# avianphysics/avian

Measured on NVIDIA H100. Metric: physics steps/sec on 100k-cube stack (broad phase + solver stage per step), higher is better.
Workload: dtype f32

## Files before the change

### avian_b200/csrc/solver_dev.cuh

```cuda
#pragma once
#include <cuda_pipeline.h>

#include "../../include/avian_b200.h"
#include "avn_math.cuh"

namespace avn {

enum { CP_N = 0, CP_T1 = 1, CP_TV = 2, CP_IDX = 3, CP_PT0 = 4, CP_PLANES = CP_PT0 + 3 * AVN_MAX_MANIFOLD_POINTS };
#define CP_ROW(k, r) (CP_PT0 + 3 * (k) + (r))
enum { CI_NP_MASK = 0x7, CI_ZERO1 = 1 << 4, CI_ZERO2 = 1 << 5, CI_NONDYN = 1 << 6, CI_TANGENT = 1 << 7,
       CI_VER1 = 1 << 8, CI_VER2 = 1 << 9 };
enum { BF_LOCK_MASK = 0x3f, BF_HAS_SOLVER_BODY = 1 << 8, BF_KINEMATIC = 1 << 9, BF_GYRO = 1 << 10, BF_DYNAMIC = 1 << 11,
       BF_CUSTOM_VEL = 1 << 12, BF_CUSTOM_POS = 1 << 13, BF_DOMINANCE_SHIFT = 16 };

enum { JP_IDX = 0,
       JP_R1 = 1,
       JP_R2 = 2,
       JP_CD = 3,
       JP_RD = 4,
       JP_A1 = 5,
       JP_A2 = 6,
       JP_B1 = 7,
       JP_B2 = 8,
       JP_LP = 9,
// ... 2 lines not shown
       JP_PLANES = 12 };

template <class S>
struct Soft { S bias, mass_scale, impulse_scale; };

template <class S>
struct DevSolver {
    int B, M, P, Mpad, J, Jpad, n_levels;
    int m_color_off[AVN_GRAPH_COLOR_COUNT + 1];
    int color_off[AVN_GRAPH_COLOR_COUNT + 1];
    int color_len[AVN_GRAPH_COLOR_COUNT];
    int wave;
    unsigned int* ver;
    int* deg;
    int* stamp;
    int substeps, iters, rest_iters, fast_trig, match_contacts;
    S h, dt, max_overlap_speed, warm_coeff, rest_threshold, joint_force_rhs;
    S gx, gy, gz;
    Soft<S> soft_dyn, soft_nondyn;
    const uint8_t* kind; const uint8_t* locked; const int8_t* dominance; const uint8_t* integ_flags;
    const S* position; const S* rotation; const S* linvel; const S* angvel; const S* inv_mass; const S* inv_inertia_local;
    const S* com; const S* lin_damp; const S* ang_damp; const S* grav_scale; const S* lin_acc; const S* ang_acc;
    const S* max_lin; const S* max_ang;
    S* out_position; S* out_rotation; S* out_linvel; S* out_angvel;
    Vec4<S>* vel; Vec4<S>* dlt; Vec4<S>* inr; Vec4<S>* itg; Vec4<S>* pre;
    const int* m_body1; const int* m_body2; const S* m_normal; const S* m_friction; const S* m_restitution; const S* m_tanvel;
    const uint32_t* m_point_begin; const uint32_t* m_point_end; const uint32_t* m_src;
    const S* p_anchor1; const S* p_anchor2; const S* p_penetration; const S* p_normal_speed;
    const S* p_ws_normal; const S* p_ws_tangent;
    const S* p_in_normal_impulse;
// ... 191 lines not shown
                                              V3<S> r1, V3<S> r2, V3<S> imp) {
    v1 = v1 - cmul(imp, in1.inv_mass);
    w1 = w1 - smul(in1.ii, cross(r1, imp));
    v2 = v2 + cmul(imp, in2.inv_mass);
    w2 = w2 + smul(in2.ii, cross(r2, imp));
}

enum { FLAG_RESTITUTION = 0, FLAG_WAVE = 1, FLAG_WORDS = 4 };
#ifdef AVN_WAVE_TRACE
#define AVN_TRACE_T(var) const long long var = clock64()
#define AVN_TRACE_ADD(d, i, v) do { if ((threadIdx.x & 31) == 0) atomicAdd(reinterpret_cast<unsigned long long*>((d).any_restitution + FLAG_WORDS) + (i), (unsigned long long)(v)); } while (0)
#else
#define AVN_TRACE_T(var)
#define AVN_TRACE_ADD(d, i, v)
#endif
__device__ __forceinline__ unsigned events_per_substep(int k, int iters) { return 2u + unsigned(2 + iters) * unsigned(k); }
enum { WV_IV = 0, WV_WARM = 1, WV_SOLVE = 2, WV_IP = 3, WV_RELAX = 4 };
__device__ __forceinline__ unsigned wave_event(int kind, int it, int s, int iters, int k, int r) {
    unsigned base = unsigned(s) * events_per_substep(k, iters);
    switch (kind) {
        case WV_IV: return base;
        case WV_WARM: return base + 1u + r;
        case WV_SOLVE: return base + 1u + unsigned(1 + it) * k + r;
        case WV_IP: return base + 1u + unsigned(1 + iters) * k;
        default: return base + 2u + unsigned(1 + iters) * k + r;
    }
}
__device__ __forceinline__ unsigned ld_acquire(const unsigned* p) {
    unsigned v;
    asm volatile("ld.acquire.gpu.global.u32 %0, [%1];" : "=r"(v) : "l"(p) : "memory");
    return v;
}
__device__ __forceinline__ void st_relaxed(unsigned* p, unsigned v) { asm volatile("st.relaxed.gpu.global.u32 [%0], %1;" ::"l"(p), "r"(v) : "memory"); }
__device__ __forceinline__ void fence_acq_rel() { asm volatile("fence.acq_rel.gpu;" ::: "memory"); }
__device__ __forceinline__ Vec4<float> ld4_cg(const Vec4<float>* p) {
    float4 v = __ldcg(reinterpret_cast<const float4*>(p));
    return mk4<float>(v.x, v.y, v.z, v.w);
}
__device__ __forceinline__ Vec4<double> ld4_cg(const Vec4<double>* p) {
    double2 a = __ldcg(reinterpret_cast<const double2*>(p)), b = __ldcg(reinterpret_cast<const double2*>(p) + 1);
// ... 18 lines not shown
    if (need2) st_relaxed(ver + b2, e2 + 1u);
}

constexpr int STAGE_ROWS = 3 * AVN_MAX_MANIFOLD_POINTS;
template <class S> __device__ __forceinline__ Vec4<S>* stage_base() {
    extern __shared__ __align__(32) unsigned char avn_stage_raw[];
    return reinterpret_cast<Vec4<S>*>(avn_stage_raw);
}
__device__ __forceinline__ void stage_copy(Vec4<float>* dst, const Vec4<float>* src) { __pipeline_memcpy_async(dst, src, 16); }
__device__ __forceinline__ void stage_copy(Vec4<double>* dst, const Vec4<double>* src) {
    __pipeline_memcpy_async(dst, src, 16);
    __pipeline_memcpy_async(reinterpret_cast<char*>(dst) + 16, reinterpret_cast<const char*>(src) + 16, 16);
}
template <class S> __host__ __device__ constexpr size_t stage_bytes(int threads, int max_points = AVN_MAX_MANIFOLD_POINTS) {
    return size_t(4 * max_points) * threads * sizeof(Vec4<S>);
}

template <class S, int PASS, int MAXP = AVN_MAX_MANIFOLD_POINTS>
__device__ __forceinline__ void contact_item(const DevSolver<S>& d, int slot) {
    const size_t MP = size_t(d.Mpad);
    Vec4<S>* c = d.cst + slot;
    Vec4<S> hidx = ld4(&c[CP_IDX * MP]);
    const int info = as_int(hidx.z);
    const int np = info & CI_NP_MASK;
    if (np == 0) return;
    const int b1 = as_int(hidx.x), b2 = as_int(hidx.y);
    Vec4<S> hn = mk4<S>(0, 0, 0, 0), ht1 = hn, htv = hn;
    BodyInertia<S> in1 = zero_inertia<S>(), in2 = zero_inertia<S>();
    Vec4<S> PC[MAXP];
    constexpr bool SOLVE = (PASS == PASS_SOLVE_BIAS || PASS == PASS_RELAX);
// ... 140 lines not shown
            if (k < np) pc_store(pc_ptr(d, k, slot), PC[k]);
    }
    if (!(info & CI_ZERO1)) {
        st4(&d.vel[2 * b1], mk4<S>(v1.x, v1.y, v1.z, S(0)));
        st4(&d.vel[2 * b1 + 1], mk4<S>(w1.x, w1.y, w1.z, S(0)));
    }
    if (!(info & CI_ZERO2)) {
        st4(&d.vel[2 * b2], mk4<S>(v2.x, v2.y, v2.z, S(0)));
        st4(&d.vel[2 * b2 + 1], mk4<S>(w2.x, w2.y, w2.z, S(0)));
    }
#undef ROW_A
#undef ROW_B
#undef ROW_D
}

template <class S, int PASS, int MAXP>
__device__ __forceinline__ void wave_contact_item(const DevSolver<S>& d, int slot, int s, int it, bool relax) {
    constexpr bool SOLVE = PASS == PASS_SOLVE_BIAS;
    relax = SOLVE && relax;
    const size_t MP = size_t(d.Mpad);
    const Vec4<S>* c = d.cst + slot;
    const Vec4<S> hidx = ld4(&c[CP_IDX * MP]);
    const int info = as_int(hidx.z);
    const int np = info & CI_NP_MASK;
    const int b1 = as_int(hidx.x), b2 = as_int(hidx.y);
    Vec4<S>* const stage = stage_base<S>() + threadIdx.x;
    const int T = blockDim.x;
#define ROW_A(k) stage[(3 * (k) + 0) * T]
#define ROW_B(k) stage[(3 * (k) + 1) * T]
#define ROW_D(k) stage[(3 * (k) + 2) * T]
#define ROW_PC(k) stage[(3 * MAXP + (k)) * T]
    Vec4<S> hn = mk4<S>(0, 0, 0, 0), ht1 = hn, htv = hn;
    BodyInertia<S> in1 = zero_inertia<S>(), in2 = zero_inertia<S>();
    if (np != 0) {
        hn = ld4(&c[CP_N * MP]);
        ht1 = ld4(&c[CP_T1 * MP]);
        if (SOLVE) htv = ld4(&c[CP_TV * MP]);
        if (!(info & CI_ZERO1)) in1 = unpack_inertia(ld4(&d.inr[2 * b1]), ld4(&d.inr[2 * b1 + 1]));
        if (!(info & CI_ZERO2)) in2 = unpack_inertia(ld4(&d.inr[2 * b2]), ld4(&d.inr[2 * b2 + 1]));
#pragma unroll 1
        for (int k = 0; k < np; ++k) {
            stage_copy(&ROW_A(k), &c[size_t(CP_ROW(k, 0)) * MP]);
            stage_copy(&ROW_B(k), &c[size_t(CP_ROW(k, 1)) * MP]);
            if (SOLVE && (info & CI_TANGENT)) stage_copy(&ROW_D(k), &c[size_t(CP_ROW(k, 2)) * MP]);
        }
    }
    __pipeline_commit();
    const bool ver1 = np != 0 && (info & CI_VER1), ver2 = np != 0 && (info & CI_VER2);
    const int rk = as_int(hidx.w);
    const int k1 = (rk >> 8) & 0xff, k2 = (rk >> 24) & 0xff;
    const int kind = SOLVE ? (relax ? WV_RELAX : WV_SOLVE) : WV_WARM;
    const unsigned e1 = wave_event(kind, it, s, d.iters, k1, rk & 0xff);
    const unsigned e2 = wave_event(kind, it, s, d.iters, k2, (rk >> 16) & 0xff);
    int* const watchdog = d.any_restitution + FLAG_WAVE;
    const V3<S> n = xyz(hn), t1 = xyz(ht1);
    const Soft<S> soft = (info & CI_NONDYN) ? d.soft_nondyn : d.soft_dyn;
    unsigned biased_points = 0;
    unsigned seen1 = 0u, seen2 = 0u;

    if (SOLVE) {
        AVN_TRACE_T(t_d0);
        const int sd = relax ? s : s - 1;
        if (sd >= 0)
            wave_wait<false>(d.ver, ver1, b1, wave_event(WV_IP, 0, sd, d.iters, k1, 0) + 1u, ver2, b2, wave_event(WV_IP, 0, sd, d.iters, k2, 0) + 1u,
                             watchdog, &seen1, &seen2);
        __pipeline_wait_prior(0);
        if (np != 0) {
            const Vec4<S> dp1 = ld4_cg(&d.dlt[2 * b1]), dq1 = ld4_cg(&d.dlt[2 * b1 + 1]);
            const Vec4<S> dp2 = ld4_cg(&d.dlt[2 * b2]), dq2 = ld4_cg(&d.dlt[2 * b2 + 1]);
            Q4<S> q1; q1.x = dq1.x; q1.y = dq1.y; q1.z = dq1.z; q1.w = dq1.w;
            Q4<S> q2; q2.x = dq2.x; q2.y = dq2.y; q2.z = dq2.z; q2.w = dq2.w;
            const V3<S> delta_translation = xyz(dp2) - xyz(dp1);
#pragma unroll
            for (int k = 0; k < MAXP; ++k) {
                if (k >= np) break;
// ... 18 lines not shown
    wave_wait(d.ver, ver1 && seen1 != e1, b1, e1, ver2 && seen2 != e2, b2, e2, watchdog);
    AVN_TRACE_ADD(d, 0, clock64() - t_w0);
    if (np == 0) return;
    AVN_TRACE_T(t_l0);
    const Vec4<S> l1 = ld4_cg(&d.vel[2 * b1]), a1 = ld4_cg(&d.vel[2 * b1 + 1]);
    const Vec4<S> l2 = ld4_cg(&d.vel[2 * b2]), a2 = ld4_cg(&d.vel[2 * b2 + 1]);
    {
        Vec4<S> pc[MAXP];
#pragma unroll
        for (int k = 0; k < MAXP; ++k)
            if (k < np) pc[k] = pc_load<true>(pc_ptr(d, k, slot));
#pragma unroll
        for (int k = 0; k < MAXP; ++k)
            if (k < np) ROW_PC(k) = pc[k];
    }
    if (!SOLVE) __pipeline_wait_prior(0);
#ifdef AVN_WAVE_TRACE
    if ((l1.x + a1.x + l2.x + a2.x) == S(1.2345e33)) d.any_restitution[1] = 2;
    AVN_TRACE_T(t_c0);
    AVN_TRACE_ADD(d, 1, t_c0 - t_l0);
#endif
    V3<S> v1 = xyz(l1), w1 = xyz(a1), v2 = xyz(l2), w2 = xyz(a2);
    const V3<S> t2 = cross(t1, n);

    if (!SOLVE) {
#pragma unroll 1
        for (int k = 0; k < np; ++k) {
            const Vec4<S> PAk = ROW_A(k), PBk = ROW_B(k), pck = ROW_PC(k);
            V3<S> r1 = xyz(PAk), r2 = xyz(PBk);
            S tx = (info & CI_TANGENT) ? pck.z : S(0), ty = (info & CI_TANGENT) ? pck.w : S(0);
            V3<S> p = d.warm_coeff * ((pck.x * n + tx * t1) + ty * t2);
            apply_impulse(v1, w1, v2, w2, in1, in2, r1, r2, p);
        }
    } else {
        const bool tangent = (info & CI_TANGENT) != 0;
#pragma unroll 1
        for (int k = 0; k < np; ++k) {
            const Vec4<S> PAk = ROW_A(k), PBk = ROW_B(k);
            Vec4<S> pck = ROW_PC(k);
            V3<S> r1 = xyz(PAk), r2 = xyz(PBk);
            V3<S> relv = (v2 + cross(w2, r2)) - (v1 + cross(w1, r1));
            S vn = dot(relv, n);
            S acc = pck.x;
            const S C = ((biased_points >> k) & 1u) ? soft.impulse_scale * acc : S(0);
            S impulse = -PBk.w * (vn + PAk.w) - C;
            S new_impulse = avn_max(acc + impulse, S(0));
            impulse = new_impulse - acc;
            pck.x = new_impulse;
            pck.y = pck.y + new_impulse;
// ... 47 lines not shown
    if (!(info & CI_ZERO2)) {
        st4(&d.vel[2 * b2], mk4<S>(v2.x, v2.y, v2.z, S(0)));
        st4(&d.vel[2 * b2 + 1], mk4<S>(w2.x, w2.y, w2.z, S(0)));
    }
    wave_publish(d.ver, ver1, b1, e1, ver2, b2, e2);
#ifdef AVN_WAVE_TRACE
    AVN_TRACE_ADD(d, 3, clock64() - t_s0);
    AVN_TRACE_ADD(d, 4, 1);
#endif
#undef ROW_A
#undef ROW_B
#undef ROW_D
#undef ROW_PC
}

template <class S, bool WAVE = false>
__device__ __forceinline__ void integrate_velocity_item(const DevSolver<S>& d, int i, int s = 0) {
    const bool in_range = i < d.B;
    int f = 0;
    if (in_range) f = as_int(ld4(&d.inr[2 * i]).y);
    const bool live = in_range && (f & BF_HAS_SOLVER_BODY);
    const bool integrate = live && !(f & BF_CUSTOM_VEL) && !(f & BF_KINEMATIC), gyro = integrate && (f & BF_GYRO);
    Vec4<S> li = mk4<S>(0, 0, 0, 0), ai = li;
    Q4<S> rot0; rot0.x = rot0.y = rot0.z = rot0.w = S(0);
    Sym3<S> il; il.m00 = il.m01 = il.m02 = il.m11 = il.m12 = il.m22 = S(0);
    if (integrate) { li = ld4(&d.itg[2 * i]); ai = ld4(&d.itg[2 * i + 1]); }
    if (gyro) {
        rot0 = ldq(d.rotation, i);
        il.m00 = d.inv_inertia_local[6 * i]; il.m01 = d.inv_inertia_local[6 * i + 1]; il.m02 = d.inv_inertia_local[6 * i + 2];
        il.m11 = d.inv_inertia_local[6 * i + 3]; il.m12 = d.inv_inertia_local[6 * i + 4]; il.m22 = d.inv_inertia_local[6 * i + 5];
    }
    const S max_lin = live && d.max_lin ? d.max_lin[i] : S(0), max_ang = live && d.max_ang ? d.max_ang[i] : S(0);
    const int bnd = live && d.bnd_of ? d.bnd_of[i] : -1;
    unsigned e = 0;
    if (WAVE) {
        if (live) e = wave_event(WV_IV, 0, s, d.iters, d.deg[i], 0);
        wave_wait(d.ver, live, i, e, false, 0, 0u, d.any_restitution + 1);
    }
    if (!live) return;
    Vec4<S> l = ldm<WAVE>(&d.vel[2 * i]), a = ldm<WAVE>(&d.vel[2 * i + 1]);
    V3<S> v = xyz(l), w = xyz(a);
    bool touched = false;
    if (integrate) {
        v = v * li.w;
        w = w * ai.w;
        v = v + xyz(li);
        w = w + xyz(ai);
        if (gyro) {
            Vec4<S> dq4 = ldm<WAVE>(&d.dlt[2 * i + 1]);
            Q4<S> dq; dq.x = dq4.x; dq.y = dq4.y; dq.z = dq4.z; dq.w = dq4.w;
            Q4<S> rot = qmul(dq, rot0);
            V3<S> lw = qrot(qconj(rot), w);
            Sym3<S> tensor = sym_inverse_or_zero(il);
            V3<S> L = smul(tensor, lw);
// ... 4 lines not shown
            } else {
                Ln = Ln * avn_sqrt(len2(L) / l2);
                w = qrot(rot, smul(il, Ln));
            }
        }
        touched = true;
    }
    if (d.max_lin) {
        S l2 = len2(v);
        if (avn_finite(max_lin) && l2 > max_lin * max_lin) { v = v * (max_lin / avn_sqrt(l2)); touched = true; }
    }
    if (d.max_ang) {
        S l2 = len2(w);
        if (avn_finite(max_ang) && l2 > max_ang * max_ang) { w = w * (max_ang / avn_sqrt(l2)); touched = true; }
    }
    if (touched) {
        st4(&d.vel[2 * i], mk4<S>(v.x, v.y, v.z, S(0)));
        st4(&d.vel[2 * i + 1], mk4<S>(w.x, w.y, w.z, S(0)));
    }
    if (bnd >= 0) {
        st4(&d.vel_ref[2 * bnd], mk4<S>(v.x, v.y, v.z, S(0)));
        st4(&d.vel_ref[2 * bnd + 1], mk4<S>(w.x, w.y, w.z, S(0)));
    }
    if (WAVE) wave_publish(d.ver, true, i, e, false, 0, 0u);
}

template <class S, bool WAVE = false>
__device__ __forceinline__ void integrate_position_item(const DevSolver<S>& d, int i, int s = 0) {
    const bool in_range = i < d.B;
    int f = 0;
    if (in_range) f = as_int(ld4(&d.inr[2 * i]).y);
    const bool live = in_range && (f & BF_HAS_SOLVER_BODY);
    unsigned e = 0;
    if (WAVE) {
        if (live) e = wave_event(WV_IP, 0, s, d.iters, d.deg[i], 0);
        wave_wait(d.ver, live, i, e, false, 0, 0u, d.any_restitution + 1);
    }
    if (!live) return;
    if (f & BF_CUSTOM_POS) {
// ... 26 lines not shown
    if (info & CI_VER1) { bad |= atomicExch(&d.stamp[b1], colour + 1) == colour + 1; r1 = atomicAdd(&d.deg[b1], 1); }
    if (info & CI_VER2) { bad |= atomicExch(&d.stamp[b2], colour + 1) == colour + 1; r2 = atomicAdd(&d.deg[b2], 1); }
    if (bad || r1 > 0xfe || r2 > 0xfe) d.any_restitution[1] = WAVE_BAD_COLOURING;
    hidx.w = int_as(S(0), (r1 & 0xff) | ((r2 & 0xff) << 16));
    st4(&c[CP_IDX * MP], hidx);
}
template <class S>
__device__ __forceinline__ void wave_pack_item(const DevSolver<S>& d, int slot) {
    const size_t MP = size_t(d.Mpad);
    Vec4<S>* c = d.cst + slot;
    Vec4<S> hidx = ld4(&c[CP_IDX * MP]);
    const int info = as_int(hidx.z);
    if ((info & CI_NP_MASK) == 0) return;
    const int b1 = as_int(hidx.x), b2 = as_int(hidx.y);
    int rk = as_int(hidx.w);
    if (info & CI_VER1) rk |= (d.deg[b1] & 0xff) << 8;
    if (info & CI_VER2) rk |= (d.deg[b2] & 0xff) << 24;
    hidx.w = int_as(S(0), rk);
    st4(&c[CP_IDX * MP], hidx);
}

template <class S>
__device__ __forceinline__ void writeback_body_item(const DevSolver<S>& d, int i) {
    Vec4<S> ia = ld4(&d.inr[2 * i]);
    int f = as_int(ia.y);
    V3<S> pos = ldv3(d.position, i);
    Q4<S> rot = ldq(d.rotation, i);
    V3<S> lv = ldv3(d.linvel, i), av = ldv3(d.angvel, i);
    if (f & BF_HAS_SOLVER_BODY) {
        Vec4<S> l = ld4(&d.vel[2 * i]), a = ld4(&d.vel[2 * i + 1]);
        Vec4<S> dp = ld4(&d.dlt[2 * i]), dq4 = ld4(&d.dlt[2 * i + 1]);
        V3<S> com = ldv3_or0(d.com, i);
        V3<S> old_com = qrot(rot, com);
        Q4<S> dq; dq.x = dq4.x; dq.y = dq4.y; dq.z = dq4.z; dq.w = dq4.w;
// ... 39 lines not shown
```

### avian_b200/csrc/solver_host.cu

```cuda
#include <algorithm>
#include <cmath>
#include <cstdlib>
#include <cstring>

#include "context.hpp"
#include "joint_schedule.hpp"
#include "solver_kernels.cuh"

namespace avn {

namespace {

template <class S>
Soft<S> softness(S damping_ratio, S hz, S delta_secs) {
    S double_damping_ratio = S(2) * damping_ratio;
    S angular_frequency = S(6.283185307179586476925286766559) * hz;
    S a1 = double_damping_ratio + angular_frequency * delta_secs;
    S a2 = angular_frequency * delta_secs * a1;
    S a3 = S(1) / (S(1) + a2);
    Soft<S> s;
    s.bias = angular_frequency / a1;
    s.mass_scale = a2 * a3;
    s.impulse_scale = a3;
    return s;
// ... 160 lines not shown
    ErrorSink* err_;
    uint32_t cfg_flags_;
    int sm_count_ = 132;
    bool coop_ok_ = false, use_mega_ = true, use_wave_ = true, l2_persist_ = false;
    size_t l2_persist_bytes_ = 0, l2_window_max_ = 0;
    int mega_grid_ = 0, mega_bps_ = 3, mega_maxp_ = 0, mega_sel_bps_ = 0;
    bool force_wave_ = false;

    template <int MAXP> const void* mega_variant(int bps) const {
        switch (bps) {
            case 2: return (const void*)step_megakernel<S, 2, MAXP>;
            case 4: return (const void*)step_megakernel<S, 4, MAXP>;
            default: return (const void*)step_megakernel<S, 3, MAXP>;
        }
    }
    static size_t mega_smem_bytes(int maxp) { return stage_bytes<S>(MEGA_BLOCK, maxp); }
    bool select_megakernel(int max_points, int bps = 0) {
        const int maxp = max_points <= 1 ? 1 : AVN_MAX_MANIFOLD_POINTS;
        if (bps == 0) bps = mega_bps_;
        if (maxp == mega_maxp_ && bps == mega_sel_bps_) return mega_grid_ > 0;
        mega_maxp_ = maxp;
        mega_sel_bps_ = bps;
        mega_fn_ = maxp == 1 ? mega_variant<1>(bps) : mega_variant<AVN_MAX_MANIFOLD_POINTS>(bps);
        const size_t smem = mega_smem_bytes(maxp);
        int per_sm = 0;
        mega_grid_ = 0;
        if (cudaFuncSetAttribute(mega_fn_, cudaFuncAttributeMaxDynamicSharedMemorySize, int(smem)) == cudaSuccess &&
            cudaOccupancyMaxActiveBlocksPerMultiprocessor(&per_sm, mega_fn_, MEGA_BLOCK, smem) == cudaSuccess && per_sm > 0)
            mega_grid_ = per_sm * sm_count_;
        else
            (void)cudaGetLastError();
// ... 369 lines not shown

        hm_ = *mc;
        if (mc->device_list) {
            host_any_restitution_ = mc->list_restitution;
        } else if (mc->reuse_graph) {
            host_any_restitution_ = graph_restitution_;
        } else {
            host_any_restitution_ = false;
            const S* r = static_cast<const S*>(mc->restitution);
            for (size_t i = 0; i < mc->M; ++i) host_any_restitution_ |= (r[i] != S(0));
            graph_restitution_ = host_any_restitution_;
        }
    }
    {
        auto up256 = [](size_t x) { return (x + 255) & ~size_t(255); };
        const size_t vel_b = up256(state_bytes), dlt_b = up256(state_bytes), ver_b = up256((B + 1) * sizeof(unsigned)), deg_b = up256(2 * (B + 1) * sizeof(int));
        const size_t planes_b = have_m_ ? size_t(CP_PLANES) * d.Mpad * sizeof(Vec4<S>) : 0;
        const size_t pcr_b = have_m_ ? up256(size_t(AVN_MAX_MANIFOLD_POINTS) * d.Mpad * sizeof(Vec4<S>)) : 0;
        AVN_CUDA(hot_.ensure(vel_b + dlt_b + ver_b + deg_b + pcr_b + planes_b + 256));
        char* base = hot_.as<char>();
        d.vel = reinterpret_cast<Vec4<S>*>(base); base += vel_b;
        d.dlt = reinterpret_cast<Vec4<S>*>(base); base += dlt_b;
        d.ver = reinterpret_cast<unsigned*>(base); base += ver_b;
        d.deg = reinterpret_cast<int*>(base); d.stamp = d.deg + (B + 1); base += deg_b;
        d.pcr = have_m_ ? reinterpret_cast<Vec4<S>*>(base) : nullptr; base += pcr_b;
        d.cst = have_m_ ? reinterpret_cast<Vec4<S>*>(base) : nullptr;
        hot_bytes_ = vel_b + dlt_b + ver_b + deg_b + pcr_b;
    }
    have_j_ = false;
    if (js) {
        size_t J = 0;
        for (int t = 0; t < AVN_JOINT_TYPE_COUNT; ++t) J += js->types[t].count;
        if (J > 0) {
            if ((st = build_joint_schedule(*bc, *js)) != AVN_OK) return st;
            have_j_ = true;
            for (int t = 0; t < AVN_JOINT_TYPE_COUNT; ++t) {
                const AvnJointColumns& jc = js->types[t];
                const size_t n = jc.count;
                const void* cols[12] = {jc.local_anchor1, jc.local_anchor2, jc.local_basis1, jc.local_basis2, jc.axis, jc.limit_min,
                                        jc.limit_max, jc.limit2_min, jc.limit2_max, jc.compliance0, jc.compliance1, jc.compliance2};
                const size_t width[12] = {3, 3, 4, 4, 3, 1, 1, 1, 1, 1, 1, 1};
// ... 69 lines not shown
    if (prepare) step_bps_ = mega_bps_;
    mega = mega && select_megakernel(max_np_, step_bps_);
    if (prepare) {
        launches_ = 0;
        cudaEventRecord(ev_[EV_RUN0], stream_);
        AVN_CUDA(cudaMemsetAsync(dev_.any_restitution, 0, FLAG_WORDS * sizeof(int) + 8 * sizeof(unsigned long long), stream_));
        int widest_colour = 0;
        for (int c = 0; c < AVN_COLOR_OVERFLOW; ++c) widest_colour = std::max(widest_colour, dev_.color_len[c]);
        const bool chain_bound = force_wave_ || widest_colour <= 2 * mega_grid_ * MEGA_BLOCK;
        dev_.wave = (mega && use_wave_ && chain_bound && dev_.M > 0 && dev_.J == 0 && dev_.color_len[AVN_COLOR_OVERFLOW] == 0) ? 1 : 0;
        if (dev_.M > 0) {
            AVN_CUDA(cudaMemsetAsync(dev_.cst + size_t(CP_IDX) * dev_.Mpad, 0, size_t(dev_.Mpad) * sizeof(Vec4<S>), stream_));
        }
        if (dev_.wave) {
            AVN_CUDA(cudaMemsetAsync(dev_.ver, 0, (size_t(dev_.B) + 1) * sizeof(unsigned), stream_));
            AVN_CUDA(cudaMemsetAsync(dev_.deg, 0, 2 * (size_t(dev_.B) + 1) * sizeof(int), stream_));
        }
        mega_step_ = mega;
    } else {
        mega = mega && mega_step_;
    }
    if (l2_persist_ && hot_bytes_ > 0) {
        cudaStreamAttrValue attr{};
        attr.accessPolicyWindow.base_ptr = hot_.p;
        attr.accessPolicyWindow.num_bytes = std::min(hot_bytes_, l2_window_max_);
        attr.accessPolicyWindow.hitRatio = float(std::min(1.0, double(l2_persist_bytes_) / double(attr.accessPolicyWindow.num_bytes)));
        attr.accessPolicyWindow.hitProp = cudaAccessPropertyPersisting;
        attr.accessPolicyWindow.missProp = cudaAccessPropertyStreaming;
        cudaStreamSetAttribute(stream_, cudaStreamAttributeAccessPolicyWindow, &attr);
    }
    const DevSolver<S>& d = dev_;
// ... 262 lines not shown
            const size_t n = hj_.types[t].count;
            if (n && dev_.jforce[t]) AVN_CUDA(cudaMemcpyAsync(hj_.types[t].force, dev_.jforce[t], 3 * n * sizeof(S), cudaMemcpyDeviceToHost, stream_));
            if (n && dev_.jtorque[t]) AVN_CUDA(cudaMemcpyAsync(hj_.types[t].torque, dev_.jtorque[t], 3 * n * sizeof(S), cudaMemcpyDeviceToHost, stream_));
        }
    }
    int flags_host[2] = {0, 0};
    AVN_CUDA(cudaMemcpyAsync(flags_host, dev_.any_restitution, sizeof flags_host, cudaMemcpyDeviceToHost, stream_));
    cudaEventRecord(ev_[EV_D2H1], stream_);
    AVN_CUDA(cudaStreamSynchronize(stream_));
#ifdef AVN_WAVE_TRACE
    {
        unsigned long long tr[8];
        cudaMemcpy(tr, dev_.any_restitution + FLAG_WORDS, sizeof tr, cudaMemcpyDeviceToHost);
        if (tr[4]) fprintf(stderr, "[avn wave trace] contact item-warps %llu  avg cycles: stage 1 (wait deltas + separations + coefficients) %.0f  wait %.0f  loads %.0f  compute %.0f  "
                           "store+publish %.0f\n", tr[4], double(tr[5]) / tr[4], double(tr[0]) / tr[4], double(tr[1]) / tr[4], double(tr[2]) / tr[4], double(tr[3]) / tr[4]);
    }
#endif
    if (flags_host[1] == WAVE_BAD_COLOURING)
        return err_->fail(AVN_ERR_INVALID_ARGUMENT, "manifolds: invalid colouring — a body with a SolverBody appears twice in one graph colour (or carries more than 254 "
                                                    "constraints): the colours are not conflict-free, the results of this step are not reliable");
    if (flags_host[1] == WAVE_WATCHDOG) return err_->fail(AVN_ERR_CUDA, "wavefront scheduler watchdog fired: results are invalid (set AVN_LAUNCH_MODE=barrier)");
    float ms = 0;
    if (cudaEventElapsedTime(&ms, ev_[EV_H2D0], ev_[EV_H2D1]) == cudaSuccess) tm_.h2d_ms = ms;
    if (cudaEventElapsedTime(&ms, ev_[EV_RUN0], ev_[EV_PREP]) == cudaSuccess) tm_.prepare_ms = ms;
    if (cudaEventElapsedTime(&ms, ev_[EV_PREP], ev_[EV_LOOP]) == cudaSuccess) tm_.substep_loop_ms = ms;
    if (cudaEventElapsedTime(&ms, ev_[EV_LOOP], ev_[EV_RUN1]) == cudaSuccess) tm_.finalize_ms = ms;
    if (cudaEventElapsedTime(&ms, ev_[EV_D2H0], ev_[EV_D2H1]) == cudaSuccess) tm_.d2h_ms = ms;
    if (cudaEventElapsedTime(&ms, ev_[EV_RUN0], ev_[EV_RUN1]) == cudaSuccess) tm_.total_ms = ms;
    tm_.kernel_launches = launches_;
    tm_.contact_constraint_count = uint32_t(dev_.M);
// ... 18 lines not shown
```

### avian_b200/csrc/solver_kernels.cuh

```cuda
#pragma once
#include <cooperative_groups.h>

#include "joints_dev.cuh"

namespace avn {
namespace cg = cooperative_groups;

constexpr int MEGA_BLOCK = 128;

enum PhaseOp {
    OP_PREPARE_BODY = 0, OP_PREPARE_CONSTRAINT, OP_PREPARE_JOINT, OP_INTEGRATE_VEL, OP_INTEGRATE_POS, OP_WARM, OP_SOLVE_BIAS,
    OP_RELAX, OP_RESTITUTION, OP_SOLVE_JOINT, OP_PROJECT_VEL, OP_DAMP_JOINT, OP_WRITEBACK_BODY, OP_STORE_IMPULSE, OP_JOINT_FORCE,
    OP_WAVE_RANK, OP_WAVE_PACK
};

template <class S, int OP, int MAXP = AVN_MAX_MANIFOLD_POINTS>
__device__ __forceinline__ void run_item(const DevSolver<S>& d, int i) {
    if (OP == OP_PREPARE_BODY) prepare_body_item(d, i);
    else if (OP == OP_PREPARE_CONSTRAINT) prepare_constraint_item(d, i);
    else if (OP == OP_PREPARE_JOINT) prepare_joint_item(d, i);
    else if (OP == OP_INTEGRATE_VEL) integrate_velocity_item(d, i);
    else if (OP == OP_INTEGRATE_POS) { integrate_position_item(d, i); if (d.J > 0) store_pre_solve_item(d, i); }
    else if (OP == OP_WARM) contact_item<S, PASS_WARM, MAXP>(d, i);
    else if (OP == OP_SOLVE_BIAS) contact_item<S, PASS_SOLVE_BIAS, MAXP>(d, i);
    else if (OP == OP_RELAX) contact_item<S, PASS_RELAX, MAXP>(d, i);
    else if (OP == OP_RESTITUTION) contact_item<S, PASS_RESTITUTION, MAXP>(d, i);
    else if (OP == OP_SOLVE_JOINT) solve_joint_item(d, i);
    else if (OP == OP_PROJECT_VEL) project_velocity_item(d, i);
    else if (OP == OP_DAMP_JOINT) damp_joint_item(d, i);
    else if (OP == OP_WRITEBACK_BODY) writeback_body_item(d, i);
    else if (OP == OP_STORE_IMPULSE) store_impulse_item(d, i);
    else if (OP == OP_JOINT_FORCE) joint_force_item(d, i);
    else if (OP == OP_WAVE_RANK) wave_rank_item(d, i);
    else if (OP == OP_WAVE_PACK) wave_pack_item(d, i);
}

template <class S, int OP>
__global__ void __launch_bounds__(256) phase_kernel(const __grid_constant__ DevSolver<S> d, int begin, int count, int serial) {
    if (serial) {
        if (blockIdx.x == 0 && threadIdx.x == 0)
            for (int i = 0; i < count; ++i) run_item<S, OP>(d, begin + i);
        return;
    }
    for (int i = blockIdx.x * blockDim.x + threadIdx.x; i < count; i += gridDim.x * blockDim.x) run_item<S, OP>(d, begin + i);
}

template <class S, int OP, int MAXP = AVN_MAX_MANIFOLD_POINTS>
__device__ __noinline__ void grid_phase(const DevSolver<S>& d, int begin, int count) {
// ... 9 lines not shown
__device__ __forceinline__ void grid_contact_pass(const DevSolver<S>& d, cg::grid_group& grid) {
    const int ov = d.color_off[AVN_COLOR_OVERFLOW], ovn = d.color_len[AVN_COLOR_OVERFLOW];
    if (ovn > 0) {
        if (blockIdx.x == 0 && threadIdx.x == 0) grid_serial<S, OP, MAXP>(d, ov, ovn);
        grid.sync();
    }
    for (int c = 0; c < AVN_COLOR_OVERFLOW; ++c) {
        const int b = d.color_off[c], n = d.color_len[c];
        if (n <= 0) continue;
        grid_phase<S, OP, MAXP>(d, b, n);
        grid.sync();
    }
}

constexpr int WAVE_CHUNK = 32;
template <class S, int PASS, int MAXP, int BPS>
__device__ __noinline__ void wave_contact_chunk(const DevSolver<S>& d, int slot, int s, int it, bool relax) {
    wave_contact_item<S, PASS, MAXP>(d, slot, s, it, relax);
}
template <class S, int BPS, int MAXP>
__device__ __noinline__ void wave_iv_chunk(const DevSolver<S>& d, int i, int s) { integrate_velocity_item<S, true>(d, i, s); }
template <class S, int BPS, int MAXP>
__device__ __noinline__ void wave_ip_chunk(const DevSolver<S>& d, int i, int s) { integrate_position_item<S, true>(d, i, s); }

template <class S, int MAXP, int BPS>
__device__ __forceinline__ void wave_substep_loop(const DevSolver<S>& d) {
    const int lane = threadIdx.x & 31;
    const long long warps = (long long)gridDim.x * (blockDim.x >> 5);
    const long long warp_id = (long long)blockIdx.x * (blockDim.x >> 5) + (threadIdx.x >> 5);
    const int body_chunks = (d.B + WAVE_CHUNK - 1) / WAVE_CHUNK, slot_chunks = d.Mpad / WAVE_CHUNK;
    const int first_chunks = body_chunks;
    const int front_passes = 1 + d.iters;
    const long long per_substep = (long long)first_chunks + body_chunks + (long long)(front_passes + 1) * slot_chunks;
    const long long total = per_substep * d.sub_end;
    for (long long g = per_substep * d.sub_begin + warp_id; g < total; g += warps) {
        const int s = int(g / per_substep);
        long long r = g - (long long)s * per_substep;
        if (r < first_chunks) {
            wave_iv_chunk<S, BPS, MAXP>(d, int(r) * WAVE_CHUNK + lane, s);
            continue;
        }
        r -= first_chunks;
        if (r < (long long)front_passes * slot_chunks) {
            const int pass = int(r / slot_chunks), slot = int(r - (long long)pass * slot_chunks) * WAVE_CHUNK + lane;
            if (pass == 0) wave_contact_chunk<S, PASS_WARM, MAXP, BPS>(d, slot, s, 0, false);
            else wave_contact_chunk<S, PASS_SOLVE_BIAS, MAXP, BPS>(d, slot, s, pass - 1, false);
            continue;
        }
        r -= (long long)front_passes * slot_chunks;
        if (r < body_chunks) { wave_ip_chunk<S, BPS, MAXP>(d, int(r) * WAVE_CHUNK + lane, s); continue; }
        r -= body_chunks;
        wave_contact_chunk<S, PASS_SOLVE_BIAS, MAXP, BPS>(d, int(r) * WAVE_CHUNK + lane, s, 0, true);
    }
}

template <class S, int BPS, int MAXP>
__global__ void __launch_bounds__(MEGA_BLOCK, BPS) step_megakernel(const __grid_constant__ DevSolver<S> d) {
    cg::grid_group grid = cg::this_grid();
    if (d.do_prepare) {
        grid_phase<S, OP_PREPARE_BODY>(d, 0, d.B + 1);
        grid.sync();
        grid_phase<S, OP_PREPARE_CONSTRAINT>(d, 0, d.M);
        grid_phase<S, OP_PREPARE_JOINT>(d, 0, d.J);
        grid.sync();
        if (d.wave) {
            for (int c = 0; c < AVN_COLOR_OVERFLOW; ++c) {
                if (d.color_len[c] <= 0) continue;
                grid_phase<S, OP_WAVE_RANK>(d, d.color_off[c], d.color_len[c]);
                grid.sync();
            }
            grid_phase<S, OP_WAVE_PACK>(d, 0, d.Mpad);
            grid.sync();
        }
    }
    const bool wave = d.wave && *reinterpret_cast<volatile int*>(d.any_restitution + 1) == 0;
    if (wave && d.sub_end > d.sub_begin) {
        wave_substep_loop<S, MAXP, BPS>(d);
        grid.sync();
    }
    for (int sub = d.sub_begin; sub < (wave ? 0 : d.sub_end); ++sub) {
        grid_phase<S, OP_INTEGRATE_VEL>(d, 0, d.B);
        grid.sync();
        if (d.M > 0) {
            grid_contact_pass<S, OP_WARM, MAXP>(d, grid);
            for (int it = 0; it < d.iters; ++it) grid_contact_pass<S, OP_SOLVE_BIAS, MAXP>(d, grid);
// ... 31 lines not shown
```

Before: 440.8.

## Fuse contact warm-start into body velocity integration via per-body adjacency lists

Result: no change. 441.1, median of 6 (+0.1%).

```diff
diff --git a/avian_b200/csrc/solver_dev.cuh b/avian_b200/csrc/solver_dev.cuh
--- a/avian_b200/csrc/solver_dev.cuh
+++ b/avian_b200/csrc/solver_dev.cuh
@@ -40,6 +40,9 @@
     unsigned int* ver;
     int* deg;
     int* stamp;
+    int* adj_cursor;
+    int* adj_off;
+    int2* adj;
     int substeps, iters, rest_iters, fast_trig, match_contacts;
     S h, dt, max_overlap_speed, warm_coeff, rest_threshold, joint_force_rhs;
     S gx, gy, gz;
@@ -261,16 +264,15 @@
 #define AVN_TRACE_T(var)
 #define AVN_TRACE_ADD(d, i, v)
 #endif
-__device__ __forceinline__ unsigned events_per_substep(int k, int iters) { return 2u + unsigned(2 + iters) * unsigned(k); }
-enum { WV_IV = 0, WV_WARM = 1, WV_SOLVE = 2, WV_IP = 3, WV_RELAX = 4 };
+__device__ __forceinline__ unsigned events_per_substep(int k, int iters) { return 2u + unsigned(1 + iters) * unsigned(k); }
+enum { WV_IV = 0, WV_SOLVE = 1, WV_IP = 2, WV_RELAX = 3 };
 __device__ __forceinline__ unsigned wave_event(int kind, int it, int s, int iters, int k, int r) {
     unsigned base = unsigned(s) * events_per_substep(k, iters);
     switch (kind) {
         case WV_IV: return base;
-        case WV_WARM: return base + 1u + r;
-        case WV_SOLVE: return base + 1u + unsigned(1 + it) * k + r;
-        case WV_IP: return base + 1u + unsigned(1 + iters) * k;
-        default: return base + 2u + unsigned(1 + iters) * k + r;
+        case WV_SOLVE: return base + 1u + unsigned(it) * k + r;
+        case WV_IP: return base + 1u + unsigned(iters) * k;
+        default: return base + 2u + unsigned(iters) * k + r;
     }
 }
 __device__ __forceinline__ unsigned ld_acquire(const unsigned* p) {
@@ -319,6 +321,15 @@
 }
 template <class S> __host__ __device__ constexpr size_t stage_bytes(int threads, int max_points = AVN_MAX_MANIFOLD_POINTS) {
     return size_t(4 * max_points) * threads * sizeof(Vec4<S>);
+}
+template <class S> __host__ __device__ constexpr int warm_bufs(int max_points) {
+    return sizeof(S) == 4 ? (max_points <= 1 ? 4 : 3) : (max_points <= 1 ? 3 : 2);
+}
+template <class S> __host__ __device__ constexpr int warm_buf_rows(int max_points) { return 2 + 2 * max_points; }
+template <class S> __host__ __device__ constexpr size_t mega_stage_bytes(int threads, int max_points) {
+    return size_t(4 * max_points > warm_bufs<S>(max_points) * warm_buf_rows<S>(max_points) ? 4 * max_points
+                                                                                             : warm_bufs<S>(max_points) * warm_buf_rows<S>(max_points)) *
+           threads * sizeof(Vec4<S>);
 }
 
 template <class S, int PASS, int MAXP = AVN_MAX_MANIFOLD_POINTS>
@@ -489,10 +500,8 @@
 #undef ROW_D
 }
 
-template <class S, int PASS, int MAXP>
+template <class S, int MAXP>
 __device__ __forceinline__ void wave_contact_item(const DevSolver<S>& d, int slot, int s, int it, bool relax) {
-    constexpr bool SOLVE = PASS == PASS_SOLVE_BIAS;
-    relax = SOLVE && relax;
     const size_t MP = size_t(d.Mpad);
     const Vec4<S>* c = d.cst + slot;
     const Vec4<S> hidx = ld4(&c[CP_IDX * MP]);
@@ -510,21 +519,21 @@
     if (np != 0) {
         hn = ld4(&c[CP_N * MP]);
         ht1 = ld4(&c[CP_T1 * MP]);
-        if (SOLVE) htv = ld4(&c[CP_TV * MP]);
+        htv = ld4(&c[CP_TV * MP]);
         if (!(info & CI_ZERO1)) in1 = unpack_inertia(ld4(&d.inr[2 * b1]), ld4(&d.inr[2 * b1 + 1]));
         if (!(info & CI_ZERO2)) in2 = unpack_inertia(ld4(&d.inr[2 * b2]), ld4(&d.inr[2 * b2 + 1]));
 #pragma unroll 1
         for (int k = 0; k < np; ++k) {
             stage_copy(&ROW_A(k), &c[size_t(CP_ROW(k, 0)) * MP]);
             stage_copy(&ROW_B(k), &c[size_t(CP_ROW(k, 1)) * MP]);
-            if (SOLVE && (info & CI_TANGENT)) stage_copy(&ROW_D(k), &c[size_t(CP_ROW(k, 2)) * MP]);
+            if (info & CI_TANGENT) stage_copy(&ROW_D(k), &c[size_t(CP_ROW(k, 2)) * MP]);
         }
     }
     __pipeline_commit();
     const bool ver1 = np != 0 && (info & CI_VER1), ver2 = np != 0 && (info & CI_VER2);
     const int rk = as_int(hidx.w);
     const int k1 = (rk >> 8) & 0xff, k2 = (rk >> 24) & 0xff;
-    const int kind = SOLVE ? (relax ? WV_RELAX : WV_SOLVE) : WV_WARM;
+    const int kind = relax ? WV_RELAX : WV_SOLVE;
     const unsigned e1 = wave_event(kind, it, s, d.iters, k1, rk & 0xff);
     const unsigned e2 = wave_event(kind, it, s, d.iters, k2, (rk >> 16) & 0xff);
     int* const watchdog = d.any_restitution + FLAG_WAVE;
@@ -533,7 +542,7 @@
     unsigned biased_points = 0;
     unsigned seen1 = 0u, seen2 = 0u;
 
-    if (SOLVE) {
+    {
         AVN_TRACE_T(t_d0);
         const int sd = relax ? s : s - 1;
         if (sd >= 0)
@@ -582,7 +591,6 @@
         for (int k = 0; k < MAXP; ++k)
             if (k < np) ROW_PC(k) = pc[k];
     }
-    if (!SOLVE) __pipeline_wait_prior(0);
 #ifdef AVN_WAVE_TRACE
     if ((l1.x + a1.x + l2.x + a2.x) == S(1.2345e33)) d.any_restitution[1] = 2;
     AVN_TRACE_T(t_c0);
@@ -591,16 +599,7 @@
     V3<S> v1 = xyz(l1), w1 = xyz(a1), v2 = xyz(l2), w2 = xyz(a2);
     const V3<S> t2 = cross(t1, n);
 
-    if (!SOLVE) {
-#pragma unroll 1
-        for (int k = 0; k < np; ++k) {
-            const Vec4<S> PAk = ROW_A(k), PBk = ROW_B(k), pck = ROW_PC(k);
-            V3<S> r1 = xyz(PAk), r2 = xyz(PBk);
-            S tx = (info & CI_TANGENT) ? pck.z : S(0), ty = (info & CI_TANGENT) ? pck.w : S(0);
-            V3<S> p = d.warm_coeff * ((pck.x * n + tx * t1) + ty * t2);
-            apply_impulse(v1, w1, v2, w2, in1, in2, r1, r2, p);
-        }
-    } else {
+    {
         const bool tangent = (info & CI_TANGENT) != 0;
 #pragma unroll 1
         for (int k = 0; k < np; ++k) {
@@ -678,12 +677,49 @@
 #undef ROW_PC
 }
 
-template <class S, bool WAVE = false>
+template <class S, bool WAVE = false, int MAXP = AVN_MAX_MANIFOLD_POINTS>
 __device__ __forceinline__ void integrate_velocity_item(const DevSolver<S>& d, int i, int s = 0) {
     const bool in_range = i < d.B;
-    int f = 0;
-    if (in_range) f = as_int(ld4(&d.inr[2 * i]).y);
+    Vec4<S> inr0 = mk4<S>(0, 0, 0, 0);
+    if (in_range) inr0 = ld4(&d.inr[2 * i]);
+    const int f = as_int(inr0.y);
     const bool live = in_range && (f & BF_HAS_SOLVER_BODY);
+    constexpr int NB = warm_bufs<S>(MAXP), WR = warm_buf_rows<S>(MAXP);
+    const size_t MP = size_t(d.Mpad);
+    Vec4<S>* const stage = stage_base<S>() + threadIdx.x;
+    const int T = blockDim.x;
+    auto skip = [](int2 c) { return (c.y & ((c.x & 1) ? CI_ZERO2 : CI_ZERO1)) != 0; };
+    auto stage_rows = [&](int j, int2 c) {
+        const int side = c.x & 1, slot = c.x >> 1, np = c.y & CI_NP_MASK;
+        if (skip(c)) return;
+        stage_copy(&stage[(j * WR + 0) * T], &d.cst[size_t(CP_N) * MP + slot]);
+        stage_copy(&stage[(j * WR + 1) * T], &d.cst[size_t(CP_T1) * MP + slot]);
+#pragma unroll 1
+        for (int kp = 0; kp < np; ++kp) stage_copy(&stage[(j * WR + 2 + kp) * T], &d.cst[size_t(CP_ROW(kp, side)) * MP + slot]);
+    };
+    auto stage_records = [&](int j, int2 c) {
+        const int slot = c.x >> 1, np = c.y & CI_NP_MASK;
+        if (skip(c)) return;
+#pragma unroll 1
+        for (int kp = 0; kp < np; ++kp) stage_copy(&stage[(j * WR + 2 + MAXP + kp) * T], pc_ptr(d, kp, slot));
+    };
+    const int k = WAVE && live ? d.deg[i] : 0;
+    const int2* const adj = d.adj + (k > 0 ? d.adj_off[i] : 0);
+    BodyInertia<S> inertia = zero_inertia<S>();
+    constexpr int NQ = 8;
+    int2 eq[NQ];
+#pragma unroll
+    for (int j = 0; j < NQ; ++j) eq[j] = make_int2(0, CI_ZERO1 | CI_ZERO2);
+    if (k > 0) {
+        inertia = unpack_inertia(inr0, ld4(&d.inr[2 * i + 1]));
+#pragma unroll
+        for (int j = 0; j < NQ; ++j)
+            if (j < k) eq[j] = adj[j];
+#pragma unroll
+        for (int j = 0; j < NB - 1; ++j)
+            if (j < k) stage_rows(j, eq[j]);
+    }
+    if (WAVE) __pipeline_commit();
     const bool integrate = live && !(f & BF_CUSTOM_VEL) && !(f & BF_KINEMATIC), gyro = integrate && (f & BF_GYRO);
     Vec4<S> li = mk4<S>(0, 0, 0, 0), ai = li;
     Q4<S> rot0; rot0.x = rot0.y = rot0.z = rot0.w = S(0);
@@ -698,10 +734,11 @@
     const int bnd = live && d.bnd_of ? d.bnd_of[i] : -1;
     unsigned e = 0;
     if (WAVE) {
-        if (live) e = wave_event(WV_IV, 0, s, d.iters, d.deg[i], 0);
+        if (live) e = wave_event(WV_IV, 0, s, d.iters, k, 0);
         wave_wait(d.ver, live, i, e, false, 0, 0u, d.any_restitution + 1);
     }
     if (!live) return;
+    AVN_TRACE_T(t_f0);
     Vec4<S> l = ldm<WAVE>(&d.vel[2 * i]), a = ldm<WAVE>(&d.vel[2 * i + 1]);
     V3<S> v = xyz(l), w = xyz(a);
     bool touched = false;
@@ -736,15 +773,59 @@
         S l2 = len2(w);
         if (avn_finite(max_ang) && l2 > max_ang * max_ang) { w = w * (max_ang / avn_sqrt(l2)); touched = true; }
     }
+    if (bnd >= 0) {
+        st4(&d.vel_ref[2 * bnd], mk4<S>(v.x, v.y, v.z, S(0)));
+        st4(&d.vel_ref[2 * bnd + 1], mk4<S>(w.x, w.y, w.z, S(0)));
+    }
+    if (WAVE && k > 0) {
+#pragma unroll
+        for (int j = 0; j < NB - 1; ++j) {
+            if (j < k) stage_records(j, eq[j]);
+            __pipeline_commit();
+        }
+#pragma unroll 1
+        for (int r = 0; r < k; ++r) {
+            if (r + NB - 1 < k) {
+                stage_rows((r + NB - 1) % NB, eq[NB - 1]);
+                stage_records((r + NB - 1) % NB, eq[NB - 1]);
+            }
+            __pipeline_commit();
+            const int2 next = r + NQ < k ? adj[r + NQ] : eq[NQ - 1];
+            __pipeline_wait_prior(NB - 1);
+            const int2 c = eq[0];
+            if (!skip(c)) {
+                const bool body2 = (c.x & 1) != 0;
+                const int info = c.y, np = info & CI_NP_MASK;
+                const Vec4<S>* const buf = stage + (r % NB) * WR * T;
+                const V3<S> n = xyz(buf[0]), t1 = xyz(buf[T]);
+                const V3<S> t2 = cross(t1, n);
+#pragma unroll
+                for (int kp = 0; kp < MAXP; ++kp) {
+                    if (kp < np) {
+                        const Vec4<S> pck = buf[(2 + MAXP + kp) * T];
+                        const V3<S> rr = xyz(buf[(2 + kp) * T]);
+                        S tx = (info & CI_TANGENT) ? pck.z : S(0), ty = (info & CI_TANGENT) ? pck.w : S(0);
+                        V3<S> p = d.warm_coeff * ((pck.x * n + tx * t1) + ty * t2);
+                        const V3<S> dv = cmul(p, inertia.inv_mass), dw = smul(inertia.ii, cross(rr, p));
+                        v = v + (body2 ? dv : -dv);
+                        w = w + (body2 ? dw : -dw);
+                    }
+                }
+                touched = true;
+            }
+#pragma unroll
+            for (int j = 0; j < NQ - 1; ++j) eq[j] = eq[j + 1];
+            eq[NQ - 1] = next;
+        }
+    }
     if (touched) {
         st4(&d.vel[2 * i], mk4<S>(v.x, v.y, v.z, S(0)));
         st4(&d.vel[2 * i + 1], mk4<S>(w.x, w.y, w.z, S(0)));
     }
-    if (bnd >= 0) {
-        st4(&d.vel_ref[2 * bnd], mk4<S>(v.x, v.y, v.z, S(0)));
-        st4(&d.vel_ref[2 * bnd + 1], mk4<S>(w.x, w.y, w.z, S(0)));
-    }
     if (WAVE) wave_publish(d.ver, true, i, e, false, 0, 0u);
+#ifdef AVN_WAVE_TRACE
+    if (WAVE) { AVN_TRACE_ADD(d, 6, clock64() - t_f0); AVN_TRACE_ADD(d, 7, 1); }
+#endif
 }
 
 template <class S, bool WAVE = false>
@@ -801,10 +882,23 @@
     if ((info & CI_NP_MASK) == 0) return;
     const int b1 = as_int(hidx.x), b2 = as_int(hidx.y);
     int rk = as_int(hidx.w);
-    if (info & CI_VER1) rk |= (d.deg[b1] & 0xff) << 8;
-    if (info & CI_VER2) rk |= (d.deg[b2] & 0xff) << 24;
+    if (info & CI_VER1) { rk |= (d.deg[b1] & 0xff) << 8; d.adj[d.adj_off[b1] + (rk & 0xff)] = make_int2(slot * 2, info); }
+    if (info & CI_VER2) { rk |= (d.deg[b2] & 0xff) << 24; d.adj[d.adj_off[b2] + ((rk >> 16) & 0xff)] = make_int2(slot * 2 + 1, info); }
     hidx.w = int_as(S(0), rk);
     st4(&c[CP_IDX * MP], hidx);
+}
+template <class S>
+__device__ __forceinline__ void wave_offset_item(const DevSolver<S>& d, int i) {
+    const int lane = threadIdx.x & 31, k = i < d.B ? d.deg[i] : 0;
+    int incl = k;
+#pragma unroll
+    for (int o = 1; o < 32; o <<= 1) {
+        const int x = __shfl_up_sync(0xffffffffu, incl, o);
+        if (lane >= o) incl += x;
+    }
+    int base = lane == 31 ? atomicAdd(d.adj_cursor, incl) : 0;
+    base = __shfl_sync(0xffffffffu, base, 31);
+    if (i < d.B) d.adj_off[i] = base + incl - k;
 }
 
 template <class S>
diff --git a/avian_b200/csrc/solver_host.cu b/avian_b200/csrc/solver_host.cu
--- a/avian_b200/csrc/solver_host.cu
+++ b/avian_b200/csrc/solver_host.cu
@@ -198,7 +198,7 @@
             default: return (const void*)step_megakernel<S, 3, MAXP>;
         }
     }
-    static size_t mega_smem_bytes(int maxp) { return stage_bytes<S>(MEGA_BLOCK, maxp); }
+    static size_t mega_smem_bytes(int maxp) { return mega_stage_bytes<S>(MEGA_BLOCK, maxp); }
     bool select_megakernel(int max_points, int bps = 0) {
         const int maxp = max_points <= 1 ? 1 : AVN_MAX_MANIFOLD_POINTS;
         if (bps == 0) bps = mega_bps_;
@@ -598,17 +598,20 @@
     }
     {
         auto up256 = [](size_t x) { return (x + 255) & ~size_t(255); };
-        const size_t vel_b = up256(state_bytes), dlt_b = up256(state_bytes), ver_b = up256((B + 1) * sizeof(unsigned)), deg_b = up256(2 * (B + 1) * sizeof(int));
+        const size_t vel_b = up256(state_bytes), dlt_b = up256(state_bytes), ver_b = up256((B + 1) * sizeof(unsigned)), deg_b = up256((3 * (B + 1) + 1) * sizeof(int));
         const size_t planes_b = have_m_ ? size_t(CP_PLANES) * d.Mpad * sizeof(Vec4<S>) : 0;
         const size_t pcr_b = have_m_ ? up256(size_t(AVN_MAX_MANIFOLD_POINTS) * d.Mpad * sizeof(Vec4<S>)) : 0;
-        AVN_CUDA(hot_.ensure(vel_b + dlt_b + ver_b + deg_b + pcr_b + planes_b + 256));
+        const size_t adj_b = have_m_ ? 2 * size_t(d.Mpad) * sizeof(int2) : 0;
+        AVN_CUDA(hot_.ensure(vel_b + dlt_b + ver_b + deg_b + pcr_b + planes_b + adj_b + 256));
         char* base = hot_.as<char>();
         d.vel = reinterpret_cast<Vec4<S>*>(base); base += vel_b;
         d.dlt = reinterpret_cast<Vec4<S>*>(base); base += dlt_b;
         d.ver = reinterpret_cast<unsigned*>(base); base += ver_b;
-        d.deg = reinterpret_cast<int*>(base); d.stamp = d.deg + (B + 1); base += deg_b;
+        d.deg = reinterpret_cast<int*>(base); d.stamp = d.deg + (B + 1); d.adj_cursor = d.stamp + (B + 1); d.adj_off = d.adj_cursor + 1;
+        base += deg_b;
         d.pcr = have_m_ ? reinterpret_cast<Vec4<S>*>(base) : nullptr; base += pcr_b;
-        d.cst = have_m_ ? reinterpret_cast<Vec4<S>*>(base) : nullptr;
+        d.cst = have_m_ ? reinterpret_cast<Vec4<S>*>(base) : nullptr; base += planes_b;
+        d.adj = have_m_ ? reinterpret_cast<int2*>(base) : nullptr;
         hot_bytes_ = vel_b + dlt_b + ver_b + deg_b + pcr_b;
     }
     have_j_ = false;
@@ -708,7 +711,7 @@
         }
         if (dev_.wave) {
             AVN_CUDA(cudaMemsetAsync(dev_.ver, 0, (size_t(dev_.B) + 1) * sizeof(unsigned), stream_));
-            AVN_CUDA(cudaMemsetAsync(dev_.deg, 0, 2 * (size_t(dev_.B) + 1) * sizeof(int), stream_));
+            AVN_CUDA(cudaMemsetAsync(dev_.deg, 0, (2 * (size_t(dev_.B) + 1) + 1) * sizeof(int), stream_));
         }
         mega_step_ = mega;
     } else {
@@ -1001,6 +1004,8 @@
         cudaMemcpy(tr, dev_.any_restitution + FLAG_WORDS, sizeof tr, cudaMemcpyDeviceToHost);
         if (tr[4]) fprintf(stderr, "[avn wave trace] contact item-warps %llu  avg cycles: stage 1 (wait deltas + separations + coefficients) %.0f  wait %.0f  loads %.0f  compute %.0f  "
                            "store+publish %.0f\n", tr[4], double(tr[5]) / tr[4], double(tr[0]) / tr[4], double(tr[1]) / tr[4], double(tr[2]) / tr[4], double(tr[3]) / tr[4]);
+        if (tr[7]) fprintf(stderr, "[avn wave trace] integrate-velocity + warm-start item-warps %llu  avg cycles after the wait (integrate, warm starts, "
+                           "store+publish) %.0f\n", tr[7], double(tr[6]) / tr[7]);
     }
 #endif
     if (flags_host[1] == WAVE_BAD_COLOURING)
diff --git a/avian_b200/csrc/solver_kernels.cuh b/avian_b200/csrc/solver_kernels.cuh
--- a/avian_b200/csrc/solver_kernels.cuh
+++ b/avian_b200/csrc/solver_kernels.cuh
@@ -11,7 +11,7 @@
 enum PhaseOp {
     OP_PREPARE_BODY = 0, OP_PREPARE_CONSTRAINT, OP_PREPARE_JOINT, OP_INTEGRATE_VEL, OP_INTEGRATE_POS, OP_WARM, OP_SOLVE_BIAS,
     OP_RELAX, OP_RESTITUTION, OP_SOLVE_JOINT, OP_PROJECT_VEL, OP_DAMP_JOINT, OP_WRITEBACK_BODY, OP_STORE_IMPULSE, OP_JOINT_FORCE,
-    OP_WAVE_RANK, OP_WAVE_PACK
+    OP_WAVE_RANK, OP_WAVE_OFFSET, OP_WAVE_PACK
 };
 
 template <class S, int OP, int MAXP = AVN_MAX_MANIFOLD_POINTS>
@@ -32,6 +32,7 @@
     else if (OP == OP_STORE_IMPULSE) store_impulse_item(d, i);
     else if (OP == OP_JOINT_FORCE) joint_force_item(d, i);
     else if (OP == OP_WAVE_RANK) wave_rank_item(d, i);
+    else if (OP == OP_WAVE_OFFSET) wave_offset_item(d, i);
     else if (OP == OP_WAVE_PACK) wave_pack_item(d, i);
 }
 
@@ -71,12 +72,12 @@
 }
 
 constexpr int WAVE_CHUNK = 32;
-template <class S, int PASS, int MAXP, int BPS>
+template <class S, int MAXP, int BPS>
 __device__ __noinline__ void wave_contact_chunk(const DevSolver<S>& d, int slot, int s, int it, bool relax) {
-    wave_contact_item<S, PASS, MAXP>(d, slot, s, it, relax);
+    wave_contact_item<S, MAXP>(d, slot, s, it, relax);
 }
 template <class S, int BPS, int MAXP>
-__device__ __noinline__ void wave_iv_chunk(const DevSolver<S>& d, int i, int s) { integrate_velocity_item<S, true>(d, i, s); }
+__device__ __noinline__ void wave_iv_chunk(const DevSolver<S>& d, int i, int s) { integrate_velocity_item<S, true, MAXP>(d, i, s); }
 template <class S, int BPS, int MAXP>
 __device__ __noinline__ void wave_ip_chunk(const DevSolver<S>& d, int i, int s) { integrate_position_item<S, true>(d, i, s); }
 
@@ -87,7 +88,7 @@
     const long long warp_id = (long long)blockIdx.x * (blockDim.x >> 5) + (threadIdx.x >> 5);
     const int body_chunks = (d.B + WAVE_CHUNK - 1) / WAVE_CHUNK, slot_chunks = d.Mpad / WAVE_CHUNK;
     const int first_chunks = body_chunks;
-    const int front_passes = 1 + d.iters;
+    const int front_passes = d.iters;
     const long long per_substep = (long long)first_chunks + body_chunks + (long long)(front_passes + 1) * slot_chunks;
     const long long total = per_substep * d.sub_end;
     for (long long g = per_substep * d.sub_begin + warp_id; g < total; g += warps) {
@@ -100,14 +101,13 @@
         r -= first_chunks;
         if (r < (long long)front_passes * slot_chunks) {
             const int pass = int(r / slot_chunks), slot = int(r - (long long)pass * slot_chunks) * WAVE_CHUNK + lane;
-            if (pass == 0) wave_contact_chunk<S, PASS_WARM, MAXP, BPS>(d, slot, s, 0, false);
-            else wave_contact_chunk<S, PASS_SOLVE_BIAS, MAXP, BPS>(d, slot, s, pass - 1, false);
+            wave_contact_chunk<S, MAXP, BPS>(d, slot, s, pass, false);
             continue;
         }
         r -= (long long)front_passes * slot_chunks;
         if (r < body_chunks) { wave_ip_chunk<S, BPS, MAXP>(d, int(r) * WAVE_CHUNK + lane, s); continue; }
         r -= body_chunks;
-        wave_contact_chunk<S, PASS_SOLVE_BIAS, MAXP, BPS>(d, int(r) * WAVE_CHUNK + lane, s, 0, true);
+        wave_contact_chunk<S, MAXP, BPS>(d, int(r) * WAVE_CHUNK + lane, s, 0, true);
     }
 }
 
@@ -126,6 +126,8 @@
                 grid_phase<S, OP_WAVE_RANK>(d, d.color_off[c], d.color_len[c]);
                 grid.sync();
             }
+            grid_phase<S, OP_WAVE_OFFSET>(d, 0, (d.B + 31) & ~31);
+            grid.sync();
             grid_phase<S, OP_WAVE_PACK>(d, 0, d.Mpad);
             grid.sync();
         }
```
